# SumitTarafder/Figbird

Measured on AMD Instinct MI355X. Metric: gaps/sec (+ filled-bases/sec), synthetic 1e5-gap set recipe, jump-library fill pass, higher is better.
Workload: dtype f64

## Files before the change

### figbird_amd/csrc/fig_abi.hip

```cpp
#include <hip/hip_runtime.h>

#include <algorithm>
#include <cstdio>
#include <cstdlib>
#include <cstring>
#include <new>
#include <vector>
#include <chrono>
#include <thread>
#include <mutex>

#include "../../include/figbird_hip.h"
#include "fig_engine.h"
#include "fig_pack.h"
#include "fig_abi_host.h"
#include "fig_quality.h"
#include "fig_quality_host.h"
#include "fig_placement.h"
#include "fig_softqual.h"
#include "fig_indel.h"
#include "fig_polish.h"

#ifdef FIG_PROF
#define FIG_PROF_BEGIN() const unsigned long long _k0 = __builtin_readcyclecounter()
// ... 370 lines not shown
    ctx->h_ins.assign(m->in_pos_dist, m->in_pos_dist + m->max_read_length);
    ctx->h_del.assign(m->del_pos_dist, m->del_pos_dist + m->max_read_length);
    std::vector<double> all;
    FigModelOffsets o;
    fig_model_tables(m, all, o, ctx->dm);
    if (ctx->d_model_tabs.p) { hipFree(ctx->d_model_tabs.p); ctx->d_model_tabs.p = nullptr; }
    if (hipMalloc(&ctx->d_model_tabs.p, all.size() * sizeof(double)) != hipSuccess) return FIG_ENOMEM;
    if (hipMemcpy(ctx->d_model_tabs.p, all.data(), all.size() * sizeof(double), hipMemcpyHostToDevice) != hipSuccess) return FIG_EHIP;
    fig_model_point(ctx->dm, o, (const double *)ctx->d_model_tabs.p);
    ctx->have_model = true;
    return FIG_OK;
}

extern "C" int64_t fig_results_capacity(const fig_model *m, const fig_gap_batch *b) {
    if (!m || !b) return FIG_EINVAL;
    return fig_pack_results_capacity(m, b);
}

enum FigKind { FIG_K_FILL, FIG_K_BEGIN, FIG_K_EVAL, FIG_K_END, FIG_K_PROBE };

template <typename... P, typename... Args>
static hipError_t launch_one(void (*k)(P...), size_t lds, int nt, int blocks, hipStream_t stream, Args... args) {
    hipError_t e = hipFuncSetAttribute((const void *)k, hipFuncAttributeMaxDynamicSharedMemorySize, (int)lds);
    if (e != hipSuccess) return e;
    hipLaunchKernelGGL(k, dim3(blocks), dim3(nt), lds, stream, args...);
    return hipGetLastError();
}

template <bool LDS_TAB, int NT>
static hipError_t launch_kind(fig_ctx *ctx, const fig_ctx::Cls &c, const FigDevBatch &db, hipStream_t stream, FigKind kind, int blocks, const void *list, int n, int qsel, int wide) {
    FigKernArgs A = fig_kargs_of(c.c, qsel, ctx->sh_on);
    if (kind == FIG_K_EVAL) { const FigKnobs &kn = ctx->fill_knobs; A.cont = kn.cont && db.cont_cap > 0; A.minc = kn.minc; A.cont_live = kn.cont_live; A.cont_prio = kn.cont_prio;
                              A.wide = A.cont ? wide : 0; A.wide_base = ctx->nslots; A.wide_cap = ctx->nslots_wide; }
    switch (kind) {
        case FIG_K_FILL: return launch_one(fig_fill_kernel<LDS_TAB, NT>, c.c.lds, NT, blocks, stream, ctx->dm, db, A);
        case FIG_K_BEGIN: return launch_one(fig_begin_kernel<LDS_TAB, NT>, c.c.lds, NT, blocks, stream, ctx->dm, db, A);
        case FIG_K_PROBE: return launch_one(fig_probe_kernel<LDS_TAB, NT>, c.c.lds, NT, blocks, stream, ctx->dm, db, A);
        case FIG_K_EVAL: return launch_one(fig_eval_kernel<LDS_TAB, NT>, c.c.lds, NT, blocks, stream, ctx->dm, db, A, (const int4 *)list, n);
        case FIG_K_END: return launch_one(fig_end_kernel<LDS_TAB, NT>, c.c.lds, NT, blocks, stream, ctx->dm, db, A, (const int *)list, n);
    }
    return hipErrorInvalidValue;
}

static hipError_t launch_any(fig_ctx *ctx, const fig_ctx::Cls &c, const FigDevBatch &db, hipStream_t stream, FigKind kind, int blocks, const void *list, int n, int qsel = 0, int wide = 0) {
    if (c.c.tiles > 0) return launch_kind<true, 512>(ctx, c, db, stream, kind, blocks, list, n, qsel, wide);
    if (c.c.lds_tab) return c.c.nt == 256 ? launch_kind<true, 256>(ctx, c, db, stream, kind, blocks, list, n, qsel, wide) : launch_kind<true, 512>(ctx, c, db, stream, kind, blocks, list, n, qsel, wide);
    return launch_kind<false, 512>(ctx, c, db, stream, kind, blocks, list, n, qsel, wide);
}

static int fig_upload_once(fig_ctx *ctx, const fig_gap_batch *b, int wide_cap, int wide_asked) {
    free_batch(ctx);
    const fig_model *m = &ctx->hm;
    hipEventRecord(ctx->ev0, ctx->stream);
    FigPacked K;
    const FigKnobs up_knobs = fig_knobs_from_env(0);
    K.nslots_wide = std::max(K.nslots, wide_cap);
    int prc = fig_pack(m, b, sizeof(FigState), K);
    if (prc) return prc;
    void *persist_mem = nullptr;
    const int wide_first = K.nslots_wide;
    K.nslots_wide = K.nslots; fig_pack_persist(K, sizeof(FigState));
    const int64_t persist_base = K.persist_total;
    K.nslots_wide = wide_first; fig_pack_persist(K, sizeof(FigState));
    size_t mem_free = 0, mem_total = 0;
    if (hipMemGetInfo(&mem_free, &mem_total) != hipSuccess) mem_free = 0;
    while (true) {
// ... 251 lines not shown
        }
        for (size_t ci = 0; ci < nc; ci++) {
            if (rcs[ci] < 0) { hipDeviceSynchronize(); return FIG_EHIP; }
            nl += rcs[ci];
            FIG_HIP(hipEventRecord(ctx->lanes[ci].done, ctx->lanes[ci].stream));
            FIG_HIP(hipStreamWaitEvent(ctx->stream, ctx->lanes[ci].done, 0));
        }
    }
    FIG_HIP(hipEventRecord(ctx->ev1, ctx->stream)); FIG_HIP(hipStreamSynchronize(ctx->stream));
    float ms = 0; FIG_HIP(hipEventElapsedTime(&ms, ctx->ev0, ctx->ev1));
    ctx->stats.kernel_ms = ms; ctx->stats.n_launches = nl;
    FIG_HIP(hipEventRecord(ctx->ev0, ctx->stream));
    std::vector<char> hstr((size_t)ctx->str_total);
    unsigned long long cnt[FIG_CNT_N] = {0};
    FIG_HIP(fetch(out->filled_len, db.filled_len, (size_t)ng * 4)); FIG_HIP(fetch(out->gaptofill, db.gaptofill, (size_t)ng * 4));
    FIG_HIP(fetch(hstr.data(), db.str, (size_t)ctx->str_total));
    FIG_HIP(fetch(cnt, db.counters, sizeof(cnt)));
    for (const FigPlane &pl : planes) FIG_HIP(fetch(pl.host, *pl.dev, pl.bytes));
    FIG_HIP(hipEventRecord(ctx->ev1, ctx->stream)); FIG_HIP(hipStreamSynchronize(ctx->stream));
    FIG_HIP(hipEventElapsedTime(&ms, ctx->ev0, ctx->ev1));
    ctx->stats.d2h_ms = ms;
#ifdef FIG_PROF
    { auto prof = [&](int i) { return cnt[i < FIG_PROF_SPLIT ? FIG_CNT_PROF_LO + i : FIG_CNT_PROF_HI + (i - FIG_PROF_SPLIT)]; };
      const unsigned long long wave = cnt[FIG_CNT_WAVE];
      const char *nm[14] = {"A.wait", "B.wait", "-", "M.finish", "PR.pre", "PR.estep", "PR.mid", "PR.mle", "PR.post", "A.chain", "A.logexp", "A.work", "B.work", "M.chains"};
      for (int i = 0; i < 14; i++) fprintf(stderr, "[figprof] %-9s %8.1f Gcycles = %5.1f %% of wave-cycles\n", nm[i], prof(i) / 1e9, wave ? 100.0 * prof(i) / wave : 0.0);
      const char *mn[4] = {"M.setup", "M.hint", "M.rounds", "M.surv"};
      for (int i = 0; i < 4; i++) fprintf(stderr, "[figprof] %-9s %8.1f Gcycles = %5.1f %% of wave-cycles\n", mn[i], prof(14 + i) / 1e9, wave ? 100.0 * prof(14 + i) / wave : 0.0);
      fprintf(stderr, "[figprof] raw slots:"); for (int i = 0; i < FIG_PROF_SLOTS; i++) fprintf(stderr, " %d:%.1f", i, prof(i) / 1e9); fprintf(stderr, "\n");
      fprintf(stderr, "[figprof] barrier wait %.3f of %.3f wave-Gcycles = %.1f %%\n", cnt[FIG_CNT_WAIT] / 1e9, wave / 1e9, wave ? 100.0 * cnt[FIG_CNT_WAIT] / wave : 0.0); }
#endif
    if (knobs.log) fprintf(stderr, "[figsched] useful flops %.4g, speculative evaluations executed %.4g (%.1f %% discarded)\n", (double)cnt[FIG_CNT_FLOPS], (double)cnt[FIG_CNT_SPEC], cnt[FIG_CNT_SPEC] ? 100.0 * (1.0 - ((double)cnt[FIG_CNT_FLOPS] / (double)cnt[FIG_CNT_SPEC])) : 0.0);
    if (knobs.log && knobs.wide) fprintf(stderr, "[figsched] widened chunks narrowed to the live workgroups: %llu\n", cnt[FIG_CNT_NARROW]);
    fig_stats_from_counters(cnt, ctx->stats);
    int rc = fig_compact_results(ng, hstr.data(), ctx->h_str_off.data(), out);
    if (!rc && sup) fig_compact_support(ng, hsup.data(), ctx->h_str_off.data(), out, sup->counts);
    return rc;
}

struct FigPostFill {
    fig_ctx *ctx = nullptr;
    const fig_gap_results *f = nullptr;
    int64_t total = 0;
    std::vector<FigDevGap> hg;
    std::vector<double> tabs;
    FigTmpBufs tmp;
    bool oom = false;
    float ms = 0;

    int open(fig_ctx *c, const fig_gap_results *filled, std::vector<double> *insd = nullptr) {
        ctx = c; f = filled;
        if (!ctx || !f || !ctx->have_batch || !ctx->have_model) return FIG_EINVAL;
        if (!f->filled_len || !f->str_off || !f->draw_pos || !f->draw_len) return FIG_EINVAL;
        hipSetDevice(ctx->device);
        const int64_t ng = ctx->n_gaps;
        if (f->str_off[0] < 0) return FIG_EINVAL;
        for (int64_t g = 0; g < ng; g++) if (f->str_off[g + 1] < f->str_off[g]) return FIG_EINVAL;
        total = f->str_off[ng];
        if (total > 0 && !f->str) return FIG_EINVAL;
        const int L = ctx->dm.L;
        hg.resize((size_t)ng);
        std::vector<double> he((size_t)L), home((size_t)L);
        tabs.resize((size_t)fig_quality_tab_doubles(L));
        if (ng > 0) FIG_HIP(fetch(hg.data(), ctx->db.gaps, (size_t)ng * sizeof(FigDevGap)));
        FIG_HIP(fetch(he.data(), ctx->dm.e, (size_t)L * sizeof(double)));
        FIG_HIP(fetch(home.data(), ctx->dm.ome1, (size_t)L * sizeof(double)));
// ... 546 lines not shown
```

### figbird_amd/csrc/fig_abi_host.h

```cpp
#ifndef FIG_ABI_HOST_H
#define FIG_ABI_HOST_H
#include <algorithm>
#include <cmath>
#include <cstdlib>
#include <cstring>
#include <vector>
#include "../../include/figbird_hip.h"
#include "fig_types.h"
#include "fig_gaprules.h"

static_assert(FIG_ORG_NONE == FIG_SUP_NONE && FIG_ORG_FINAL == FIG_SUP_FINAL && FIG_ORG_ORIGINAL == FIG_SUP_ORIGINAL && FIG_ORG_TIEBREAK == FIG_SUP_TIEBREAK,
              "the engine's path mask (fig_types.h) is fig_gap_support::origin");

static inline const char *fig_strerror_text(int code) {
    switch (code) {
        case FIG_OK: return "ok";
        case FIG_EINVAL: return "invalid argument";
        case FIG_ENODEV: return "no usable HIP device (libfighip has no CPU path)";
        case FIG_ENOMEM: return "out of memory";
        case FIG_EHIP: return "HIP runtime error";
        case FIG_ENOSPC: return "result string buffer too small";
        case FIG_EUNSUP: return "input outside the supported envelope";
        default: return "unknown error";
    }
// ... 120 lines not shown
    for (int64_t g = 0; g < ng; g++) {
        out->str_off[g] = o;
        int n = out->filled_len[g];
        if (n > 0) { memcpy(out->str + o, src + src_off[g], (size_t)n); o += n; }
    }
    out->str_off[ng] = o;
    return FIG_OK;
}

static void fig_compact_support(int64_t ng, const int32_t *src, const int64_t *src_off, const fig_gap_results *out, int32_t *dst) {
    for (int64_t g = 0; g < ng; g++) {
        int n = out->filled_len[g];
        if (n > 0) memcpy(dst + out->str_off[g] * 5, src + src_off[g] * 5, (size_t)n * 5 * sizeof(int32_t));
    }
}

static int fig_fill_gaps_once(fig_ctx *ctx, const fig_gap_batch *batch, fig_gap_results *out) {
    int rc = fig_batch_upload(ctx, batch);
    if (rc) return rc;
    rc = fig_fill_resident(ctx, out);
    fig_batch_free(ctx);
    return rc;
}

struct FigKnobs {
    bool seq;
    bool cont; int cont_cap, cont_live, cont_prio;
    int wide, slots_wide, wide_max_active;
    bool lanes_serial;
    bool log;
    int minc;
    double ipw;
    int sh_on;
};

#define FIG_WIDE_DEFAULT_UNMAPPED FIG_WIDE_GROW
#define FIG_SLOTS_WIDE_MAX 4096
static FigKnobs fig_knobs_from_env(int unmapped) {
    FigKnobs k;
    const char *sched = getenv("FIG_SCHED"), *ser = getenv("FIG_LANES"), *mc = getenv("FIG_MIN_CHUNK"), *ipw = getenv("FIG_ITEMS_PER_WG");
    const char *ev = getenv("FIG_ESTEP"), *sc = getenv("FIG_SH_CHUNKS");
    k.seq = sched && strcmp(sched, "seq") == 0;
    const char *cc = getenv("FIG_CONT_CAP"), *cl = getenv("FIG_CONT_LIVE"), *cp = getenv("FIG_CONT_PRIO");
    k.cont = sched ? strcmp(sched, "continuous") == 0 : unmapped != 0;
    k.cont_cap = cc ? std::max(1, atoi(cc)) : FIG_CONT_CAP_MAX;
    k.cont_live = cl ? std::max(0, atoi(cl)) : 100;
    k.cont_prio = cp ? (atoi(cp) != 0) : 1;
    const char *wd = getenv("FIG_WIDE"), *sw = getenv("FIG_SLOTS_WIDE");
    k.wide = !wd ? (unmapped ? FIG_WIDE_DEFAULT_UNMAPPED : 0) : !strcmp(wd, "grow") ? FIG_WIDE_GROW : !strcmp(wd, "idle") ? FIG_WIDE_IDLE : !strcmp(wd, "both") ? (FIG_WIDE_GROW | FIG_WIDE_IDLE) : 0;
    if (!k.cont) k.wide = 0;
    k.slots_wide = sw ? atoi(sw) : 256;
    const char *wa = getenv("FIG_WIDE_MAX_ACTIVE");
    k.wide_max_active = wa ? std::max(0, atoi(wa)) : 96;
    k.lanes_serial = ser && strcmp(ser, "serial") == 0;
    k.log = getenv("FIG_SCHED_LOG") != nullptr;
    k.minc = mc ? std::max(1, atoi(mc)) : 16;
    k.ipw = ipw ? std::max(1.0, atof(ipw)) : (unmapped ? 12.0 : 6.0);
    k.sh_on = (ev && !strcmp(ev, "pair")) ? 0 : (sc ? std::max(1, std::min(FIG_SH_SC, atoi(sc))) : FIG_SH_SC);
    return k;
}

struct FigRound { std::vector<FigItem> items; std::vector<FigEntry> entries; int chunk = 0, n_active = 0; };

static inline int fig_wide_for_lane(int wide_mode, int n_active_max, int wide_max_active) {
    return n_active_max > wide_max_active ? (wide_mode & ~FIG_WIDE_GROW) : wide_mode;
}

static void fig_plan_round(const std::vector<int> &ids, const FigGapCtl *ctl, int capacity, int nsplit, int slots_cap, int wide_mode, int wide_cap, int wide_max_active, int minc, double ipw_base,
                           int &n_active_max, FigRound &R) {
    R.items.clear(); R.entries.clear();
    R.chunk = 0; R.n_active = 0;
    for (int g : ids) if (ctl[g].status == FIG_GAP_MORE) R.n_active++;
    if (R.n_active == 0) return;
    long long rem_total = 0;
    for (int g : ids) if (ctl[g].status == FIG_GAP_MORE) rem_total += std::max(0, ctl[g].range - ctl[g].j);
    n_active_max = std::max(n_active_max, R.n_active);
    wide_mode = fig_wide_for_lane(wide_mode, n_active_max, wide_max_active);
    const double ipw = ipw_base * std::min(8.0, std::max(1.0, n_active_max / 96.0));
    const double share = rem_total > 0 ? (ipw * capacity / (double)std::max(1, nsplit)) / (double)rem_total : 1.0;
    const double target = ipw * capacity / (double)std::max(1, nsplit);
    long long total = 0;
    for (int g : ids) {
        if (ctl[g].status != FIG_GAP_MORE) continue;
        if ((double)total >= 1.25 * target) break;
        int j = ctl[g].j, range = ctl[g].range;
        int want = (int)std::ceil((range - j) * share);
        want = std::min(std::max(want, minc), slots_cap);
        int n = std::max(0, std::min(want, range - j));
        if (j > 0 && n > 0 && (wide_mode & FIG_WIDE_GROW) && wide_cap > slots_cap)
            n = std::max(n, fig_wide_chunk(FigWide{FIG_WIDE_GROW, slots_cap, wide_cap}, 1, ctl[g].last, wide_cap, range - j, 1, 0));
        total += n;
// ... 41 lines not shown
```

### figbird_amd/csrc/fig_engine.h

```cpp
#ifndef FIG_ENGINE_H
#define FIG_ENGINE_H

#include "fig_types.h"

#ifdef FIG_EMU
#include <cmath>
#include <cstring>
#define FIG_D static inline
#define FIG_NOINLINE
#define FIG_HD static inline
#define FIG_SYNC() ((void)0)
FIG_D double fig_log10(double x) { return log10(x); }
FIG_D double fig_log(double x) { return log(x); }
FIG_D double fig_exp(double x) { return exp(x); }
FIG_D double fig_pow10(double x) { return pow(10, x); }
FIG_D int fig_atomic_add_i32(int *p, int v) { int o = *p; *p += v; return o; }
FIG_D void fig_atomic_max_i32(int *p, int v) { if (v > *p) *p = v; }
FIG_D int fig_atomic_fetch_add_i32(int *p, int v) { int o = *p; *p += v; return o; }
FIG_D void fig_atomic_min_i32(int *p, int v) { if (v < *p) *p = v; }
FIG_D void fig_atomic_or_i32(int *p, int v) { *p |= v; }
FIG_D void fig_atomic_add_u64(unsigned long long *p, unsigned long long v) { *p += v; }
FIG_D unsigned long long fig_shfl_down_u64(unsigned long long v, int off) { (void)v; (void)off; return 0; }
#else
#include <hip/hip_runtime.h>
#define FIG_D __device__ static
#define FIG_NOINLINE __attribute__((noinline))
#define FIG_HD __host__ __device__ static
#ifdef FIG_PROF
#define FIG_SYNC() do { unsigned long long _bt = __builtin_readcyclecounter(); __syncthreads(); E.wait_cycles += __builtin_readcyclecounter() - _bt; } while (0)
#else
#define FIG_SYNC() __syncthreads()
#endif
FIG_D double fig_log10(double x) { return log10(x); }
FIG_D double fig_log(double x) { return log(x); }
FIG_D double fig_exp(double x) { return exp(x); }
FIG_D double fig_pow10(double x) { return pow(10.0, x); }
FIG_D int fig_atomic_add_i32(int *p, int v) { return atomicAdd(p, v); }
FIG_D void fig_atomic_max_i32(int *p, int v) { atomicMax(p, v); }
FIG_D int fig_atomic_fetch_add_i32(int *p, int v) { return atomicAdd(p, v); }
FIG_D void fig_atomic_min_i32(int *p, int v) { atomicMin(p, v); }
FIG_D void fig_atomic_or_i32(int *p, int v) { atomicOr(p, v); }
FIG_D void fig_atomic_add_u64(unsigned long long *p, unsigned long long v) { atomicAdd(p, v); }
FIG_D unsigned long long fig_shfl_down_u64(unsigned long long v, int off) { return __shfl_down(v, off, 64); }
#endif

#define FIG_NOPOS 0x7fffffff
#define FIG_PLB_TEAMS 8
#define FIG_PLB_BYTES (FIG_PLB_TEAMS * 64 * 4)

#if defined(FIG_PROF) && !defined(FIG_EMU)
#define FIG_T0(E) unsigned long long _fig_t = __builtin_readcyclecounter()
#define FIG_TICK(E, slot) do { unsigned long long _n = __builtin_readcyclecounter(); (E).prof[slot] += _n - _fig_t; _fig_t = _n; } while (0)
#define FIG_COUNT(E, slot, n) do { (E).prof[slot] += (n); } while (0)
#else
#define FIG_COUNT(E, slot, n) do { } while (0)
#define FIG_T0(E) do { } while (0)
#define FIG_TICK(E, slot) do { } while (0)
#endif

#ifdef FIG_EMU
static double *fig_lds = nullptr;
#define FIG_RFL(x) (x)
typedef const uint32_t *fig_cu32p;
typedef const double *fig_cdp;
typedef double *fig_gdp;
typedef const double *fig_gcdp;
typedef const uint32_t *fig_gcu32p;
typedef const unsigned char *fig_gcu8p;
typedef const unsigned char *fig_lcu8p;
#else
extern __shared__ __attribute__((aligned(16))) double fig_lds[];
#define FIG_RFL(x) __builtin_amdgcn_readfirstlane(x)
typedef const uint32_t __attribute__((address_space(4))) *fig_cu32p;
typedef const double __attribute__((address_space(4))) *fig_cdp;
typedef double __attribute__((address_space(1))) *fig_gdp;
typedef const double __attribute__((address_space(1))) *fig_gcdp;
typedef const uint32_t __attribute__((address_space(1))) *fig_gcu32p;
typedef const unsigned char __attribute__((address_space(1))) *fig_gcu8p;
typedef const unsigned char __attribute__((address_space(3))) *fig_lcu8p;
#endif

// ... 47 lines not shown
struct FigTrip { int v[3]; };



struct FigScr {
    double *cnt;
    double *ncnt;
    double *tmp;
    int *pc;
    int *nci;
    unsigned char *accf;
    unsigned char *mdone;
    int *cov;
    int *region;
    unsigned char *cons, *best, *cur, *prev, *orig;
    unsigned char *colchar;
    unsigned char *mark, *saved;
    double *maxlv;
    int *frp;
    int *org;
    int *fin;
    FigTrip *sortbuf;
    int *hint;
    int *hint_e;
    double *hval;
    int *repeatflag;
    int *ppos_org;
    int *pflag;
    int *prf;
    int *lcross, *rcross; unsigned char *smflag;
    int *used_read_arr; int *lrmd;
    FigPQ *pqg; double *q4g;
    double *wg;
};

FIG_HD long long fig_align8(long long x) { return (x + 15) & ~15LL; }

FIG_HD long long fig_scratch_layout(unsigned char *base, int capG, int capR, int capP, int capC, int capW, int capE, FigScr *s) {
    long long o = 0;
#define FIG_CARVE(field, type, count) do { if (s) s->field = (type *)(base + o); o = fig_align8(o + (long long)sizeof(type) * (count)); } while (0)
    FIG_CARVE(cnt, double, 5LL * capG);
    FIG_CARVE(ncnt, double, 5LL * capG);
    FIG_CARVE(tmp, double, 5LL * capG);
    FIG_CARVE(pqg, FigPQ, 4LL * capE);
    FIG_CARVE(q4g, double, capE);
    FIG_CARVE(wg, double, capW);
    FIG_CARVE(maxlv, double, capR > capP ? capR : capP);
    FIG_CARVE(hval, double, capR);
    FIG_CARVE(pc, int, 4LL * capG);
    FIG_CARVE(nci, int, 5LL * capG);
    FIG_CARVE(cov, int, capG);
    FIG_CARVE(region, int, 2LL * capG + 16);
    FIG_CARVE(frp, int, 2LL * capR);
    FIG_CARVE(org, int, 2LL * capR);
    FIG_CARVE(fin, int, 2LL * capR);
    FIG_CARVE(sortbuf, FigTrip, capR);
    FIG_CARVE(hint, int, capR);
    FIG_CARVE(hint_e, int, capR);
    FIG_CARVE(repeatflag, int, 3LL * capP);
    FIG_CARVE(ppos_org, int, 3LL * capP);
    FIG_CARVE(pflag, int, 2LL * capP);
    FIG_CARVE(prf, int, 3LL * capP);
    FIG_CARVE(lcross, int, capP);
    FIG_CARVE(rcross, int, capP);
    FIG_CARVE(used_read_arr, int, capC);
    FIG_CARVE(lrmd, int, 2LL * capC);
    FIG_CARVE(cons, unsigned char, capG + 8);
    FIG_CARVE(best, unsigned char, capG + 8);
    FIG_CARVE(cur, unsigned char, capG + 8);
    FIG_CARVE(prev, unsigned char, capG + 8);
    FIG_CARVE(orig, unsigned char, capG + 8);
    FIG_CARVE(colchar, unsigned char, capG + 8);
    FIG_CARVE(mark, unsigned char, capR + 8);
    FIG_CARVE(saved, unsigned char, capR + 8);
    FIG_CARVE(accf, unsigned char, capR + 8);
    FIG_CARVE(mdone, unsigned char, capR + 8);
    FIG_CARVE(smflag, unsigned char, capP + 8);
#undef FIG_CARVE
    return o;
}

struct FigEng {
    int tid, nt;
    const FigDevModel *M;
    const FigDevBatch *B;
    const FigDevGap *g;
    FigState *S;
    FigScr scr;
    FigPQ *pq; double *q4;
    int ncolE, xoff;
    int off_pq, off_q4, off_w;
    int off_plb;
    int pq_lds, w_lds;
    int lds_tw;
    int tiles, tile_step, tile_cols;
    double *wbuf;
    int Wcap, nteams;
    int sh_on;
    int lane, wave, nw, wsz;
    const double *kt_fwd, *kt_rev;
    const double *mt_fwd, *mt_rev;
    unsigned char *rb;
    uint32_t *plb;
    unsigned char *gs;
    int capG;
    unsigned long long flops;
    unsigned long long mle_alg;
    unsigned long long mle_exec;
    unsigned long long wait_cycles;
    unsigned long long prof[FIG_PROF_SLOTS];
};

FIG_D void fig_eng_ident(FigEng &E, unsigned tid, unsigned nt, unsigned wsz) {
    E.tid = (int)tid; E.nt = (int)nt;
    E.lane = (int)(tid % wsz); E.wave = (int)(tid / wsz); E.nw = (int)((nt + wsz - 1) / wsz); E.wsz = (int)wsz;
}

struct FigKernArgs { int capG, capGl, ncolE, Wcap, nteams, q_begin, q_end, qsel, tiles, tile_step, tile_cols, tiled_max, sh_on;
                     int cont = 0, minc = 16, cont_live = 100, cont_prio = 1;
                     int wide = 0, wide_base = 64, wide_cap = 64; };

FIG_D long long fig_eng_carve(FigEng &E, const FigDevModel &M, const FigKernArgs &A, bool lds_tab) {
    E.capG = A.capG;
    E.ncolE = A.ncolE; E.xoff = M.L - 1; E.Wcap = A.Wcap; E.nteams = A.nteams; E.sh_on = A.sh_on;
    long long off = 0;
    E.pq_lds = lds_tab; E.w_lds = lds_tab;
    E.tiles = A.tiles; E.tile_step = A.tile_step; E.tile_cols = A.tile_cols;
    if (lds_tab && A.tiles > 0) {
        E.pq_lds = 0;
        E.off_pq = 0; E.off_q4 = 8 * A.tile_cols; E.off_w = 9 * A.tile_cols;
        off = 9LL * A.tile_cols + (long long)A.nteams * A.Wcap;
        { const long long mle = FIG_TILED_MLE_DOUBLES(A.ncolE, (int)E.nw); if (mle > off && mle <= A.tiled_max) off = mle; }
        E.pq = E.scr.pqg; E.q4 = E.scr.q4g; E.wbuf = E.scr.wg;
    } else if (lds_tab) {
        E.off_pq = 0; E.off_q4 = 8 * A.ncolE; E.off_w = 9 * A.ncolE;
        off = 9LL * A.ncolE + (long long)A.nteams * A.Wcap;
        E.pq = (FigPQ *)(fig_lds + E.off_pq); E.q4 = fig_lds + E.off_q4; E.wbuf = fig_lds + E.off_w;
    } else {
        E.off_pq = E.off_q4 = E.off_w = 0;
        E.pq = E.scr.pqg; E.q4 = E.scr.q4g; E.wbuf = E.scr.wg;
    }
    E.S = (FigState *)(fig_lds + off); E.lds_tw = (int)off;
    unsigned char *bp = (unsigned char *)(E.S + 1);
    E.gs = bp; bp += ((A.capGl + 7) & ~7);
    E.rb = bp; bp += ((FIG_MAX_READLEN + 8 + 15) & ~15);
    E.plb = (uint32_t *)bp; E.off_plb = (int)((double *)bp - fig_lds);
    E.kt_fwd = M.ome; E.kt_rev = M.ome + 2 * M.L; E.mt_fwd = M.ome + 4 * M.L; E.mt_rev = M.ome + 6 * M.L;
    return off * 8 + (long long)sizeof(FigState) + ((A.capGl + 7) & ~7) + ((FIG_MAX_READLEN + 8 + 15) & ~15) + FIG_PLB_BYTES;
}

FIG_D int fig_read_code(const uint32_t *packed, long long woff, int len, int j) {
    int nw2 = (len + 15) >> 4;
    uint32_t w = packed[woff + (j >> 4)];
    uint32_t m = packed[woff + nw2 + (j >> 5)];
    int c = (w >> ((j & 15) * 2)) & 3;
    return ((m >> (j & 31)) & 1) ? 4 : c;
}
// ... 317 lines not shown
```

### figbird_amd/csrc/fig_engine_core.h

```cpp

struct FigWin { int lo, hi; int tis0; int dir; };

FIG_D FigWin fig_window_unmapped(const FigEng &E, int pos1, int len, int G, int gapoffset) {
    const FigDevModel &M = *E.M;
    long long gsl = E.g->gapStart;
    FigWin w;
    int lo = -(len - 1), hi = G - 1;
    if ((long long)pos1 < gsl) {
        w.tis0 = (int)(gsl - pos1 + len); w.dir = 1;
        int a = M.Tmin - w.tis0, b = M.Tmax - w.tis0;
        if (a > lo) lo = a;
        if (b < hi) hi = b;
    } else {
        int p = pos1 + gapoffset;
        w.tis0 = (int)(p - gsl + len); w.dir = -1;
        int a = w.tis0 - M.Tmax, b = w.tis0 - M.Tmin;
        if (a > lo) lo = a;
        if (b < hi) hi = b;
    }
    w.lo = lo; w.hi = hi;
    return w;
}

FIG_D FigWin fig_window_partial(const FigEng &E, int pos1, int ref_pos, int len, int G, int gapoffset, int shift_always) {
// ... 270 lines not shown
        if (found != -1) {
            int remn = s2n - s4n;
            int part_count = 0;
            for (int p = 0; p < np; p++) {
                unsigned char rs[FIG_MAX_READLEN + 8];
                int len = fig_load_read(E, E.B->p, E.g->pBase + p, rs);
                int max_match = -1, max_pos = -1;
                if (len >= s1n) {
                    for (int j = 0; j < len - s1n; j++) {
                        int mc = 0, mm = 0;
                        for (int kk = 0; kk < s1n; kk++) { if (rs[j + kk] == S.gap_left[kk]) mc++; else mm++; if (mm > 2) break; }
                        if (mc > max_match) { max_match = mc; max_pos = j; }
                    }
                }
                if (s1n - max_match <= 2) {
                    int newpos = max_pos + s1n, match = 0;
                    for (int j = 0; j < remn; j++) {
                        int rc = (newpos + j < len) ? rs[newpos + j] : 255;
                        if (S.gap_right[s4n + j] == rc) match++;
                    }
                    if (remn - match <= 2) return s4n;
                }
                part_count++;
                if (part_count > FIG_READ_CAP) break;
            }
        }
    }
    return 0;
}

FIG_D int fig_initialize(FigEng &E, int gl, int negGapCheck) {
    FigState &S = *E.S;
    int cg = E.capG;
    if (E.tid == 0) { S.G = gl; fig_ise(E); S.region_perct = 0; }
    FIG_SYNC();
    int G = S.G;
    for (int x = E.tid; x < cg; x += E.nt) {
        if (x < G) { E.scr.cnt[x] = 0; E.scr.cnt[cg + x] = 0; E.scr.cnt[2 * cg + x] = 0; E.scr.cnt[3 * cg + x] = 0; E.scr.cnt[4 * cg + x] = 1;
                     for (int j = 0; j < 5; j++) E.scr.ncnt[j * cg + x] = 0; }
        for (int j = 0; j < 5; j++) E.scr.tmp[j * cg + x] = 0;
        E.scr.cov[x] = 0;
    }
    int nml = E.g->nU > E.g->nP ? E.g->nU : E.g->nP;
    for (int r = E.tid; r < nml; r += E.nt) E.scr.maxlv[r] = 0;
    for (int r = E.tid; r < E.g->nU; r += E.nt) { E.scr.hint[r] = FIG_NOPOS; E.scr.hint_e[r] = FIG_NOPOS; }
    FIG_SYNC();
    if (E.tid == 0) {
        int gfp = 0;
        if (S.side_limit > 0 && negGapCheck == 0) gfp = fig_find_contig_match(E);
        S.bc_i = gfp;
    }
    FIG_SYNC();
    int gfp = S.bc_i;
    fig_compute_probs(E);
    FIG_SYNC();
    fig_update_partial_prob(E, G);
    fig_compute_errprobs_only(E);
    FIG_SYNC();
    return gfp;
}

FIG_D double fig_get_diff(const unsigned char *target, const unsigned char *ref, int length) {
    double diff = 0;
    for (int i = 0; i < length; i++) if (target[i] != ref[i]) diff++;
    return diff / length;
}
FIG_D int fig_find_partial_match(const unsigned char *ref, int len_r, const unsigned char *search, int len_s, int pos, int c, int len_t) {
// ... 265 lines not shown
            }
        }
    }
    if (flag1 == 1 && num_match_count0 == 0 && index_pair[0] < S.pl_len) {
        for (int f = index_pair[0] + 1; f < S.pl_len; f++) if (f < G) count_pos[S.partial_left[f] * cg + f] += 1;
    }
    for (int j = 0; j < G; j++) {
        int total_count_p = 0;
        for (int k = 0; k < 4; k++) total_count_p += count_pos[k * cg + j];
        if (total_count_p > 0) for (int k = 0; k < 4; k++) E.scr.cnt[k * cg + j] = (count_pos[k * cg + j] / total_count_p);
    }
}

#include "fig_engine_hot.h"
#include "fig_engine_partial.h"

FIG_D void fig_dbg_planes(FigEng &E, int nreads) {
    const FigDevBatch &B = *E.B;
    if (!B.dbg_counts && !B.dbg_read_maxlv) return;
    FIG_SYNC();
    const int j = E.S->dbg_j;
    if (j >= 0 && j < B.dbg_max_cand) {
        const long long rec = (long long)E.g->gapNo * B.dbg_max_cand + j;
        if (B.dbg_counts) {
            int n = E.S->ncols < B.dbg_plane_cols ? E.S->ncols : B.dbg_plane_cols;
            double *dst = B.dbg_counts + rec * B.dbg_plane_cols * 5;
            for (int x = E.tid; x < n; x += E.nt) for (int b = 0; b < 5; b++) dst[(long long)x * 5 + b] = E.scr.cnt[b * E.capG + x];
        }
        if (B.dbg_read_maxlv) {
            int n = nreads < B.dbg_plane_reads ? nreads : B.dbg_plane_reads;
            double *dst = B.dbg_read_maxlv + rec * B.dbg_plane_reads;
            for (int r = E.tid; r < n; r += E.nt) dst[r] = E.scr.maxlv[r];
        }
    }
    FIG_SYNC();
}

template <bool LDS>
FIG_D void fig_place_reads(FigEng &E, int ge, int finalize_flag, int gapoffset, int updateflag) {
    FigState &S = *E.S;
    const FigDevModel &M = *E.M;
    int cg = E.capG, G = S.G, left = S.left, right = S.right;
    int nU = E.g->nU, G0 = E.g->G0;
    if (E.tid == 0) S.n_place++;
    FIG_T0(E);
    for (int x = E.tid; x < S.ncols; x += E.nt) for (int j = 0; j < 5; j++) E.scr.cnt[j * cg + x] = 0;
    for (int r = E.tid; r < nU; r += E.nt) {
        E.scr.maxlv[r] = 0; E.scr.mark[r] = 0; E.scr.frp[r * 2] = -200; E.scr.frp[r * 2 + 1] = 0;
        if (G == G0) { E.scr.org[r * 2] = -200; E.scr.org[r * 2 + 1] = 0; }
    }
    for (int r = E.tid; r < S.partial_read_count; r += E.nt) E.scr.maxlv[r] = 0;
    if (E.tid == 0) S.lik = 0;
    FIG_SYNC();
    double maxLikelihood = 0;

    if (M.partial_flag) {
        int np = E.g->nP;
        int nproc = np < FIG_READ_CAP ? np : FIG_READ_CAP;
        const FigDevReads &PR = E.B->p;
        long long pb = E.g->pBase;
        unsigned char *const rb_keep = E.rb; double *const wbuf_keep = E.wbuf;
        unsigned long long pfl = 0, pml = 0;
        int nrow = E.nw < FIG_PLB_TEAMS ? E.nw : FIG_PLB_TEAMS;
        long long rstride = 208;
        if ((long long)nrow * rstride > (long long)E.nteams * E.Wcap) { nrow = E.nw < E.nteams ? E.nw : E.nteams; if (nrow > FIG_PLB_TEAMS) nrow = FIG_PLB_TEAMS; rstride = E.Wcap; }
        if (nrow < 1) nrow = 1;
// ... 113 lines not shown
                double temp_log_val = -fig_log10(best.v);
                if (temp_log_val < M.cutoff) {
                    fig_atomic_add_i32(&S.valid_count, 1);
                    E.scr.pflag[p * 2 + 1] = o;
                    if (G == G0) { E.scr.ppos_org[p * 3] = 1; E.scr.ppos_org[p * 3 + 1] = o; E.scr.ppos_org[p * 3 + 2] = len; }
                } else { fig_atomic_add_i32(&S.invalid_count, 1); E.scr.pflag[p * 2] = 0; }
            }
        }
        E.rb = rb_keep;
        FIG_TICK(E, 33);
        E.flops += pfl; E.mle_alg += pml;
        { unsigned long long t = pml; for (int off = 32; off > 0; off >>= 1) t += fig_shfl_down_u64(t, off); E.mle_exec += t; }
        FIG_SYNC();
        FIG_TICK(E, 5);
        int ret_val[2] = {0, 0};
        fig_detect_overlap_par<LDS>(E, E.scr.pflag, 2, G, ret_val, 8);
        if (E.tid == 0) {
            if (ret_val[0] == 300) maxLikelihood += ret_val[0];
            else if (ret_val[0] >= 1 && ret_val[0] < FIG_MAX_READLEN) maxLikelihood += 30 * ret_val[0];
            else if (ret_val[1] == -1) maxLikelihood += -100;
        }
        FIG_SYNC();
    }

    if (M.unmapped == 1) {
        FIG_TICK(E, 4);
        fig_hot_estep_dispatch<LDS>(E, gapoffset);
        FIG_TICK(E, 5);
        fig_dbg_planes(E, nU);
        fig_compute_sequence(E, 0, 0);
        for (int x = E.tid; x < S.ncols; x += E.nt) E.gs[x] = E.scr.cons[x];
        FIG_SYNC();
        FIG_TICK(E, 6);
        fig_mle_dispatch<LDS>(E, gapoffset, 0, G, left, right);
        FIG_TICK(E, 7);
        for (int x = E.tid; x < S.ncols; x += E.nt) for (int j = 0; j < 5; j++) E.scr.ncnt[j * cg + x] = (double)E.scr.nci[j * cg + x];
        if (E.tid < E.wsz) {
            for (int r0 = 0; r0 < nU; r0 += E.wsz) {
                const int r = r0 + E.lane;
                double term = 0;
                if (r < nU) term = E.scr.accf[r] ? E.scr.maxlv[r] : -50.0;
                const int n = nU - r0 < E.wsz ? nU - r0 : E.wsz;
#ifdef FIG_EMU
                for (int k = 0; k < n; k++) maxLikelihood += term;
#else
                long long bits; memcpy(&bits, &term, 8);
                const int lo32 = (int)(bits & 0xffffffffLL), hi32 = (int)(bits >> 32);
                for (int k = 0; k < n; k++) {
                    const unsigned int l = (unsigned int)__builtin_amdgcn_readlane(lo32, k), h = (unsigned int)__builtin_amdgcn_readlane(hi32, k);
                    const long long b2 = (long long)(((unsigned long long)h << 32) | l);
                    double t; memcpy(&t, &b2, 8);
                    maxLikelihood += t;
                }
#endif
            }
        }
        FIG_SYNC();
        fig_compute_sequence(E, 1, 1);
        if (E.tid == 0) { S.ibuf[0] = (S.cons_len == S.prev_len) ? 1 : 0; }
        FIG_SYNC();
        if (S.ibuf[0]) {
            int neq = 0;
            for (int x = E.tid; x < S.cons_len; x += E.nt) if (E.scr.cons[x] != E.scr.prev[x]) neq = 1;
            if (neq) S.ibuf[0] = 0;
        }
        FIG_SYNC();
        int same = S.ibuf[0];
        FIG_SYNC();
        if (same) { if (E.tid == 0) S.comp_count++; }
// ... 425 lines not shown
```

### figbird_amd/csrc/fig_types.h

```cpp
#ifndef FIG_TYPES_H
#define FIG_TYPES_H
#include <stdint.h>

#define FIG_MAX_READLEN 200
#define FIG_READ_CAP 3000
#define FIG_MAX_GAP 100000
#define FIG_FLANK 208
#define FIG_DBL_MAX 1.7976931348623157e308
#define FIG_SH_C 32
#define FIG_SH_SC 4
#define FIG_SH_ONE 16
#define FIG_MLE_FB 208
#define FIG_TILED_MLE_DOUBLES(ncolE, nw) (7LL * (ncolE) + (long long)(nw) * FIG_MLE_FB + ((ncolE) + 15) / 16 + 16 + 8)

enum { FIG_ORG_NONE = 0, FIG_ORG_FINAL = 1, FIG_ORG_ORIGINAL = 2, FIG_ORG_TIEBREAK = 4 };

enum { FIG_GAP_FINISHED = 0, FIG_GAP_MORE = 1, FIG_GAP_LOOP_DONE = 2 };
struct FigGapCtl { int32_t status, j, range; union { int32_t reach; int32_t last; }; };

struct alignas(16) FigItem { int32_t gap, j, slot, chunk; };
struct alignas(16) FigEntry { int32_t gap, n, j_planned, stamped; };
static_assert(sizeof(FigGapCtl) == 16 && sizeof(FigItem) == 16 && sizeof(FigEntry) == 16, "control words are four int32: buffers and copies are sized by sizeof");
enum { FIG_CONT_EVAL = 0, FIG_CONT_END = 1 };
#define FIG_CONT_CAP_MAX 65535
struct alignas(16) FigCont { int32_t gap, j0, n, kind; int32_t next, ready, rank, pad; };
struct alignas(16) FigContHdr { int32_t tail, exited, open, pad; };
static_assert(sizeof(FigCont) == 32 && sizeof(FigContHdr) == 16, "continuation records: buffers are sized by sizeof");

enum FigCounter {
    FIG_CNT_PLACE = 0,
    FIG_CNT_FLOPS = 1, FIG_CNT_SPEC = 2,
    FIG_CNT_MLE_ALG = 3, FIG_CNT_MLE_EXEC = 4,
    FIG_CNT_CONT = 5,
    FIG_CNT_NARROW = 6,
    FIG_CNT_PROF_LO = 8, FIG_CNT_WAIT = 30, FIG_CNT_WAVE = 31, FIG_CNT_PROF_HI = 32,
    FIG_CNT_N = 64
};
#define FIG_PROF_SLOTS 40
#define FIG_PROF_SPLIT 22

struct FigDevModel {
    int32_t L;
    int32_t Tmin, Tmax, cutoff;
    int32_t partial_flag, unmapped, script_itr, D, read_length, neg_overlap, partial_len, unm_limit;
    int32_t max_insert;
    double T[25];
    const double *e;
    const double *ome;
    const double *ome1;
    const double *m3;
    const double *insd;
    const double *qtab;
    double fmm_up;
};

struct FigDevGap {
    int64_t gapStart, contigLen;
    int32_t G0, stat2, stat3, fillflag;
    int32_t nU; int32_t nP;
    int64_t uBase, pBase;
    int32_t alloc_arg; float gpf1, gpf2; int32_t lgf;
    int64_t flankOff;
    int64_t strOff;
    int32_t gapNo; int32_t cls;
    int64_t persistOff;
    int32_t capGg, rangeCap, nslots, pad;
    int64_t streamOff;
};
// ... 38 lines not shown
```

Measured before the change: 26.21.

## Memoize MLE placement pass when gap key and consensus are unchanged

Adds a per-gap cache of the maximum-likelihood read placement results, keyed by G, left/right bounds, column count, gap offset and the consensus string. When a later iteration of the fill loop hits the same key, it restores the accepted flags, max-likelihood values, read positions and valid counts instead of rerunning the MLE dispatch. The goal is to skip redundant placeReads work in unmapped-read mode. In exchange it needs extra scratch carving, a consensus comparison pass with additional barriers, and correctness relies on the key fully capturing the MLE inputs. The ncnt refresh is skipped on the reuse path.

```diff
diff --git a/figbird_amd/csrc/fig_abi.hip b/figbird_amd/csrc/fig_abi.hip
--- a/figbird_amd/csrc/fig_abi.hip
+++ b/figbird_amd/csrc/fig_abi.hip
@@ -426,6 +426,7 @@
     FigKernArgs A = fig_kargs_of(c.c, qsel, ctx->sh_on);
     if (kind == FIG_K_EVAL) { const FigKnobs &kn = ctx->fill_knobs; A.cont = kn.cont && db.cont_cap > 0; A.minc = kn.minc; A.cont_live = kn.cont_live; A.cont_prio = kn.cont_prio;
                               A.wide = A.cont ? wide : 0; A.wide_base = ctx->nslots; A.wide_cap = ctx->nslots_wide; }
+    if (kind != FIG_K_PROBE) A.mle_reuse = ctx->fill_knobs.mle_reuse;
     switch (kind) {
         case FIG_K_FILL: return launch_one(fig_fill_kernel<LDS_TAB, NT>, c.c.lds, NT, blocks, stream, ctx->dm, db, A);
         case FIG_K_BEGIN: return launch_one(fig_begin_kernel<LDS_TAB, NT>, c.c.lds, NT, blocks, stream, ctx->dm, db, A);
@@ -743,6 +744,7 @@
 #endif
     if (knobs.log) fprintf(stderr, "[figsched] useful flops %.4g, speculative evaluations executed %.4g (%.1f %% discarded)\n", (double)cnt[FIG_CNT_FLOPS], (double)cnt[FIG_CNT_SPEC], cnt[FIG_CNT_SPEC] ? 100.0 * (1.0 - ((double)cnt[FIG_CNT_FLOPS] / (double)cnt[FIG_CNT_SPEC])) : 0.0);
     if (knobs.log && knobs.wide) fprintf(stderr, "[figsched] widened chunks narrowed to the live workgroups: %llu\n", cnt[FIG_CNT_NARROW]);
+    if (knobs.log && knobs.mle_reuse) fprintf(stderr, "[figsched] MLE passes reused: %llu of %llu placeReads calls executed (%.1f %%)\n", cnt[FIG_CNT_MLE_REUSED], cnt[FIG_CNT_MLE_ASKED], cnt[FIG_CNT_MLE_ASKED] ? 100.0 * (double)cnt[FIG_CNT_MLE_REUSED] / (double)cnt[FIG_CNT_MLE_ASKED] : 0.0);
     fig_stats_from_counters(cnt, ctx->stats);
     int rc = fig_compact_results(ng, hstr.data(), ctx->h_str_off.data(), out);
     if (!rc && sup) fig_compact_support(ng, hsup.data(), ctx->h_str_off.data(), out, sup->counts);
diff --git a/figbird_amd/csrc/fig_abi_host.h b/figbird_amd/csrc/fig_abi_host.h
--- a/figbird_amd/csrc/fig_abi_host.h
+++ b/figbird_amd/csrc/fig_abi_host.h
@@ -176,6 +176,7 @@
     int minc;
     double ipw;
     int sh_on;
+    int mle_reuse;
 };
 
 #define FIG_WIDE_DEFAULT_UNMAPPED FIG_WIDE_GROW
@@ -201,6 +202,8 @@
     k.minc = mc ? std::max(1, atoi(mc)) : 16;
     k.ipw = ipw ? std::max(1.0, atof(ipw)) : (unmapped ? 12.0 : 6.0);
     k.sh_on = (ev && !strcmp(ev, "pair")) ? 0 : (sc ? std::max(1, std::min(FIG_SH_SC, atoi(sc))) : FIG_SH_SC);
+    const char *mr = getenv("FIG_MLE_REUSE");
+    k.mle_reuse = unmapped != 0 && !(mr && !strcmp(mr, "0"));
     return k;
 }
 
diff --git a/figbird_amd/csrc/fig_engine.h b/figbird_amd/csrc/fig_engine.h
--- a/figbird_amd/csrc/fig_engine.h
+++ b/figbird_amd/csrc/fig_engine.h
@@ -47,6 +47,7 @@
 #define FIG_NOPOS 0x7fffffff
 #define FIG_PLB_TEAMS 8
 #define FIG_PLB_BYTES (FIG_PLB_TEAMS * 64 * 4)
+enum FigMrKey { FIG_MR_G = 0, FIG_MR_LEFT, FIG_MR_RIGHT, FIG_MR_NCOLS, FIG_MR_GAPOFF, FIG_MR_VALID, FIG_MR_VCOUNT, FIG_MR_KEYS = 8 };
 
 #if defined(FIG_PROF) && !defined(FIG_EMU)
 #define FIG_T0(E) unsigned long long _fig_t = __builtin_readcyclecounter()
@@ -160,6 +161,12 @@
     int *used_read_arr; int *lrmd;
     FigPQ *pqg; double *q4g;
     double *wg;
+    unsigned char *mr_gs;
+    unsigned char *mr_acc;
+    double *mr_maxlv;
+    int *mr_frp;
+    int *mr_key;
+    unsigned long long *mr_credit;
 };
 
 FIG_HD long long fig_align8(long long x) { return (x + 15) & ~15LL; }
@@ -204,6 +211,12 @@
     FIG_CARVE(accf, unsigned char, capR + 8);
     FIG_CARVE(mdone, unsigned char, capR + 8);
     FIG_CARVE(smflag, unsigned char, capP + 8);
+    FIG_CARVE(mr_maxlv, double, capR);
+    FIG_CARVE(mr_credit, unsigned long long, 16);
+    FIG_CARVE(mr_frp, int, 2LL * capR);
+    FIG_CARVE(mr_key, int, FIG_MR_KEYS);
+    FIG_CARVE(mr_gs, unsigned char, capG + 8);
+    FIG_CARVE(mr_acc, unsigned char, capR + 8);
 #undef FIG_CARVE
     return o;
 }
@@ -225,6 +238,7 @@
     double *wbuf;
     int Wcap, nteams;
     int sh_on;
+    int mle_reuse;
     int lane, wave, nw, wsz;
     const double *kt_fwd, *kt_rev;
     const double *mt_fwd, *mt_rev;
@@ -246,11 +260,12 @@
 
 struct FigKernArgs { int capG, capGl, ncolE, Wcap, nteams, q_begin, q_end, qsel, tiles, tile_step, tile_cols, tiled_max, sh_on;
                      int cont = 0, minc = 16, cont_live = 100, cont_prio = 1;
-                     int wide = 0, wide_base = 64, wide_cap = 64; };
+                     int wide = 0, wide_base = 64, wide_cap = 64;
+                     int mle_reuse = 0; };
 
 FIG_D long long fig_eng_carve(FigEng &E, const FigDevModel &M, const FigKernArgs &A, bool lds_tab) {
     E.capG = A.capG;
-    E.ncolE = A.ncolE; E.xoff = M.L - 1; E.Wcap = A.Wcap; E.nteams = A.nteams; E.sh_on = A.sh_on;
+    E.ncolE = A.ncolE; E.xoff = M.L - 1; E.Wcap = A.Wcap; E.nteams = A.nteams; E.sh_on = A.sh_on; E.mle_reuse = A.mle_reuse;
     long long off = 0;
     E.pq_lds = lds_tab; E.w_lds = lds_tab;
     E.tiles = A.tiles; E.tile_step = A.tile_step; E.tile_cols = A.tile_cols;
diff --git a/figbird_amd/csrc/fig_engine_core.h b/figbird_amd/csrc/fig_engine_core.h
--- a/figbird_amd/csrc/fig_engine_core.h
+++ b/figbird_amd/csrc/fig_engine_core.h
@@ -326,7 +326,7 @@
 FIG_D int fig_initialize(FigEng &E, int gl, int negGapCheck) {
     FigState &S = *E.S;
     int cg = E.capG;
-    if (E.tid == 0) { S.G = gl; fig_ise(E); S.region_perct = 0; }
+    if (E.tid == 0) { S.G = gl; fig_ise(E); S.region_perct = 0; if (E.mle_reuse) E.scr.mr_key[FIG_MR_VALID] = 0; }
     FIG_SYNC();
     int G = S.G;
     for (int x = E.tid; x < cg; x += E.nt) {
@@ -658,6 +658,62 @@
             double *dst = B.dbg_read_maxlv + rec * B.dbg_plane_reads;
             for (int r = E.tid; r < n; r += E.nt) dst[r] = E.scr.maxlv[r];
         }
+    }
+    FIG_SYNC();
+}
+
+FIG_D bool fig_mle_reuse_on(const FigEng &E) { return E.mle_reuse && E.M->fmm_up <= 1.0 && !E.M->partial_flag; }
+
+FIG_D bool fig_mle_reuse_probe(FigEng &E, int gapoffset) {
+    FigState &S = *E.S;
+    const int *key = E.scr.mr_key;
+    if (E.tid == 0) S.ibuf[0] = key[FIG_MR_VALID] == 1 && key[FIG_MR_G] == S.G && key[FIG_MR_LEFT] == S.left && key[FIG_MR_RIGHT] == S.right &&
+                                key[FIG_MR_NCOLS] == S.ncols && key[FIG_MR_GAPOFF] == gapoffset;
+    FIG_SYNC();
+    int neq = 0;
+    for (int x = E.tid; x < S.ncols; x += E.nt) { const unsigned char c = E.gs[x]; if (E.scr.mr_gs[x] != c) { neq = 1; E.scr.mr_gs[x] = c; } }
+    if (neq) S.ibuf[0] = 0;
+    FIG_SYNC();
+    const int same = S.ibuf[0];
+    FIG_SYNC();
+    if (E.tid == 0) { fig_atomic_add_u64(&E.B->counters[FIG_CNT_MLE_ASKED], 1ull); if (same) fig_atomic_add_u64(&E.B->counters[FIG_CNT_MLE_REUSED], 1ull); }
+    return same != 0;
+}
+
+FIG_D void fig_mle_reuse_keep(FigEng &E, int gapoffset, unsigned long long alg, int vc0) {
+    FigState &S = *E.S;
+    for (int r = E.tid; r < E.g->nU; r += E.nt) {
+        const unsigned char a = E.scr.accf[r];
+        E.scr.mr_acc[r] = a;
+        if (a) { E.scr.mr_maxlv[r] = E.scr.maxlv[r]; E.scr.mr_frp[r * 2] = E.scr.frp[r * 2]; E.scr.mr_frp[r * 2 + 1] = E.scr.frp[r * 2 + 1]; }
+    }
+    for (int off = 32; off > 0; off >>= 1) alg += fig_shfl_down_u64(alg, off);
+    if (E.lane == 0) E.scr.mr_credit[E.wave] = alg;
+    if (E.tid == 0) {
+        int *key = E.scr.mr_key;
+        key[FIG_MR_G] = S.G; key[FIG_MR_LEFT] = S.left; key[FIG_MR_RIGHT] = S.right; key[FIG_MR_NCOLS] = S.ncols; key[FIG_MR_GAPOFF] = gapoffset;
+        key[FIG_MR_VCOUNT] = S.valid_count - vc0; key[FIG_MR_VALID] = 1;
+    }
+}
+
+FIG_D void fig_mle_reuse_restore(FigEng &E) {
+    FigState &S = *E.S;
+    const bool at_g0 = S.G == E.g->G0;
+    for (int r = E.tid; r < E.g->nU; r += E.nt) {
+        const unsigned char a = E.scr.mr_acc[r];
+        E.scr.accf[r] = a;
+        if (a) {
+            const int of = E.scr.mr_frp[r * 2], len = E.scr.mr_frp[r * 2 + 1];
+            E.scr.maxlv[r] = E.scr.mr_maxlv[r]; E.scr.mark[r] = 1;
+            E.scr.frp[r * 2] = of; E.scr.frp[r * 2 + 1] = len;
+            if (at_g0) { E.scr.org[r * 2] = of; E.scr.org[r * 2 + 1] = len; }
+        }
+    }
+    if (E.tid == 0) {
+        unsigned long long alg = 0;
+        for (int w = 0; w < E.nw; w++) alg += E.scr.mr_credit[w];
+        E.flops += alg; E.mle_alg += alg;
+        S.valid_count += E.scr.mr_key[FIG_MR_VCOUNT];
     }
     FIG_SYNC();
 }
@@ -837,9 +893,18 @@
         for (int x = E.tid; x < S.ncols; x += E.nt) E.gs[x] = E.scr.cons[x];
         FIG_SYNC();
         FIG_TICK(E, 6);
-        fig_mle_dispatch<LDS>(E, gapoffset, 0, G, left, right);
-        FIG_TICK(E, 7);
-        for (int x = E.tid; x < S.ncols; x += E.nt) for (int j = 0; j < 5; j++) E.scr.ncnt[j * cg + x] = (double)E.scr.nci[j * cg + x];
+        const bool reuse = fig_mle_reuse_on(E);
+        if (reuse && fig_mle_reuse_probe(E, gapoffset)) {
+            fig_mle_reuse_restore(E);
+            FIG_TICK(E, 7);
+        } else {
+            const unsigned long long alg0 = E.mle_alg;
+            const int vc0 = S.valid_count;
+            fig_mle_dispatch<LDS>(E, gapoffset, 0, G, left, right);
+            FIG_TICK(E, 7);
+            if (reuse) fig_mle_reuse_keep(E, gapoffset, E.mle_alg - alg0, vc0);
+            for (int x = E.tid; x < S.ncols; x += E.nt) for (int j = 0; j < 5; j++) E.scr.ncnt[j * cg + x] = (double)E.scr.nci[j * cg + x];
+        }
         if (E.tid < E.wsz) {
             for (int r0 = 0; r0 < nU; r0 += E.wsz) {
                 const int r = r0 + E.lane;
diff --git a/figbird_amd/csrc/fig_types.h b/figbird_amd/csrc/fig_types.h
--- a/figbird_amd/csrc/fig_types.h
+++ b/figbird_amd/csrc/fig_types.h
@@ -34,6 +34,7 @@
     FIG_CNT_CONT = 5,
     FIG_CNT_NARROW = 6,
     FIG_CNT_PROF_LO = 8, FIG_CNT_WAIT = 30, FIG_CNT_WAVE = 31, FIG_CNT_PROF_HI = 32,
+    FIG_CNT_MLE_ASKED = 50, FIG_CNT_MLE_REUSED = 51,
     FIG_CNT_N = 64
 };
 #define FIG_PROF_SLOTS 40
```

Result: faster. 27.99, median of 6 (+6.8%).
